# UbiquitousLearning/Mandheling-DSP-Training

Measured on AMD Instinct MI355X. Metric: training images/sec + int8 MFMA TOPS, VGG-11 batch 256, 1/2/4/8 MI355X, higher is better.
Workload: dtype int8; 1 GPU; VGG11 NITI int8 training step (fwd+relu+pool, loss grad, weight grad, input grad, SGD), 3x32x32; global_batch=256, per_gpu_batch=256, parallelism=single GPU, streams=one stream (weight gradient, then input gradient, per layer)

## Files before the change

include/niti_hip.h:

```cpp
#ifndef NITI_HIP_H
#define NITI_HIP_H

#include <stddef.h>
#include <stdint.h>

#ifdef __cplusplus
extern "C" {
#endif

enum niti_error_code {
    NITI_NO_ERROR = 0,
    NITI_OUT_OF_MEMORY = 1,
    NITI_NOT_SUPPORT = 2,
    NITI_COMPUTE_SIZE_ERROR = 3,
    NITI_NO_EXECUTION = 4,
    NITI_INVALID_VALUE = 5,
    NITI_INPUT_DATA_ERROR = 10,
    NITI_CALL_BACK_STOP = 11
};

enum niti_op_type {
    NITI_OP_CONV_INT8 = 700,
    NITI_OP_DECONV_INT8 = 701,
    NITI_OP_RELU_INT8 = 703,
// ... 157 lines not shown
    int8_t* out_p16;
    int8_t* pool3_out;
    int8_t* pool3_arg;
    int relu, pool_relu, pool_h, pool_w;
    int zero_cls, zc_h, zc_w;
    int pool3_h, pool3_w, pool3_oh, pool3_ow;
} niti_requant_fused;
int niti_requant_act_fused(const int32_t* acc, int64_t rows, int ldc, const uint32_t* amax,
                           const niti_requant_fused* f, void* stream);
int niti_requant_grad(const int32_t* acc, int64_t n, const uint32_t* amax, int rule, int8_t* g_out,
                      int8_t* w_update, void* stream);
int niti_sgd_update(const int32_t* acc, const uint32_t* amax, int rule, int co, int ci, int kk, int cip, int cop,
                    int8_t* w_ohwi16, int8_t* wt_ihwo16, int8_t* g_out, void* stream);
int niti_sgd_update_wf(const int32_t* acc, const uint32_t* amax, int rule, int co, int ci, int kk, int cip, int cop,
                       int8_t* w_ohwi16, int8_t* wt_ihwo16, int8_t* g_out, int8_t* wf, int8_t* wft, void* stream);
int niti_nhwc16_to_chwn16(const int8_t* in, int n, int hw, int cp, int np, int8_t* out, void* stream);
int niti_ohwi16_to_ihwo16(const int8_t* w, int co, int ci, int kk, int cip, int cop, int8_t* wt, void* stream);
int niti_nchw_to_nhwc16(const int8_t* x, int n, int c, int hw, int cp, int8_t* out, void* stream);
int niti_nchw_to_chwn16(const int8_t* x, int n, int c, int hw, int cp, int np, int8_t* out, void* stream);
int niti_nhwc16_to_nchw(const int8_t* x, int n, int c, int hw, int cp, int8_t* out, void* stream);
int niti_oihw_to_ohwi16(const int8_t* w, int co, int ci, int kk, int cip, int8_t* out, void* stream);
int niti_ohwi16_to_oihw(const int8_t* w, int co, int ci, int kk, int cip, int8_t* out, void* stream);
int niti_residual_add(const int8_t* a, const int8_t* ea, const int8_t* b, const int8_t* eb, int64_t n, int32_t* z,
                      int8_t* ez, uint32_t* amax, void* stream);
int niti_residual_requant(const int8_t* a, const int8_t* ea, const int8_t* b, const int8_t* eb, int64_t n,
                          const uint32_t* amax, int8_t* ez, int8_t* exp_out, int relu, int8_t* out, void* stream);
int niti_residual_requant_relu_grad(const int8_t* a, const int8_t* ea, const int8_t* b, const int8_t* eb, int64_t n,
                                    const uint32_t* amax, int8_t* ez, int8_t* exp_out, const int8_t* relu_mask,
                                    int8_t* out, void* stream);
int niti_sum_pool(const int8_t* x, int n, int hw, int cp, int32_t* acc, uint32_t* amax, void* stream);
// ... 121 lines not shown
```

mandheling-dsp-training_amd/csrc/niti_capi.hip:

```cpp
#include "../../include/niti_hip.h"
#include <memory>
#include <vector>

#include "niti_internal.hpp"
#include "niti_kernels.hpp"

struct niti_execution {
    niti::Execution* impl = nullptr;
    int op = 0;
    std::vector<void*> stage;
    std::vector<size_t> stage_bytes;
    uint32_t* err_host = nullptr;
    ~niti_execution() {
        delete impl;
        for (void* p : stage)
            if (p) (void)hipFree(p);
        if (err_host) (void)hipHostFree(err_host);
    }
};

namespace {
int code(hipError_t e) {
    if (e == hipSuccess) return NITI_NO_ERROR;
    if (e == hipErrorOutOfMemory) return NITI_OUT_OF_MEMORY;
// ... 577 lines not shown
int niti_sgd_update(const int32_t* acc, const uint32_t* amax, int rule, int co, int ci, int kk, int cip, int cop,
                    int8_t* w, int8_t* wt, int8_t* g_out, void* stream) {
    if (rule != 2 && rule != 3) return NITI_INVALID_VALUE;
    return code(niti::sgd_update(acc, amax, rule, co, ci, kk, cip, cop, w, wt, g_out, S(stream)));
}
int niti_sgd_update_wf(const int32_t* acc, const uint32_t* amax, int rule, int co, int ci, int kk, int cip, int cop,
                       int8_t* w, int8_t* wt, int8_t* g_out, int8_t* wf, int8_t* wft, void* stream) {
    if (rule != 2 && rule != 3) return NITI_INVALID_VALUE;
    if ((wf || wft) && (kk != 9 || ci % 32 != 0 || co % 32 != 0)) return NITI_NOT_SUPPORT;
    niti::SgdJob j{acc, amax, rule, co, ci, kk, cip, cop, w, wt, g_out};
    j.wf = wf;
    j.wft = wft;
    return code(niti::sgd_update_many(&j, 1, S(stream)));
}

int niti_nhwc16_to_chwn16(const int8_t* in, int n, int hw, int cp, int np, int8_t* out, void* stream) {
    return code(niti::nhwc16_to_chwn16(in, n, hw, cp, np, out, S(stream)));
}
int niti_ohwi16_to_ihwo16(const int8_t* w, int co, int ci, int kk, int cip, int cop, int8_t* wt, void* stream) {
    return code(niti::ohwi16_to_ihwo16(w, co, ci, kk, cip, cop, wt, S(stream)));
}
int niti_nchw_to_nhwc16(const int8_t* x, int n, int c, int hw, int cp, int8_t* out, void* stream) {
    return code(niti::nchw_to_nhwc16(x, n, c, hw, cp, out, S(stream)));
}
int niti_nchw_to_chwn16(const int8_t* x, int n, int c, int hw, int cp, int np, int8_t* out, void* stream) {
    return code(niti::nchw_to_chwn16(x, n, c, hw, cp, np, out, S(stream)));
}
int niti_nhwc16_to_nchw(const int8_t* x, int n, int c, int hw, int cp, int8_t* out, void* stream) {
    return code(niti::nhwc16_to_nchw(x, n, c, hw, cp, out, S(stream)));
}
// ... 215 lines not shown
```

mandheling-dsp-training_amd/csrc/niti_kernels.hip:

```cpp
#include <stdlib.h>

#include <map>
#include <atomic>
#include <mutex>
#include <type_traits>
#include <vector>
#include <algorithm>
#include <stdio.h>

#include <hip/hip_ext.h>

#include "niti_device.hpp"
#include "niti_gridbar.hpp"
#include "niti_kernels.hpp"
#include "niti_sgd.hpp"
#include "niti_map.hpp"

namespace niti {


bool ConvGeom::finalize() {
    if (n <= 0 || c_in <= 0 || h <= 0 || w <= 0 || c_out <= 0 || kh <= 0 || kw <= 0) return false;
    if (sh <= 0 || sw <= 0 || dh <= 0 || dw <= 0) return false;
    const int keh = dh * (kh - 1) + 1, kew = dw * (kw - 1) + 1;
// ... 1666 lines not shown

template <class LA, class LB, bool KT = false>
static hipError_t gemm_acc_plan(const GemmPlan& p, const LA& la, const LB& lb, int M, int N, int kc_total, int32_t* C,
                                uint32_t* amax, int32_t* ws, hipStream_t st, hipEvent_t after_gemm = nullptr,
                                SgdJob* defer = nullptr) {
    Epi e;
    if (KT) e.span = take_span();
    if (p.strat == STRAT_SLAB) {
        e.C = ws;
        e.ldc = N;
        e.slab_stride = (int64_t)slab_stride_elems(M, N);
        if (const char* f = getenv("NITI_DIAG_SPLIT_MAJOR")) e.split_major = atoi(f);
        hipError_t r = launch_mode<LA, LB, EPI_SLAB, KT>(p, la, lb, M, N, kc_total, e, st);
        if (r == hipSuccess && after_gemm != nullptr) r = hipEventRecord(after_gemm, st);
        if (r != hipSuccess) return r;
        if (defer != nullptr && ((int64_t)M * N) % 4 == 0 && (int64_t)M * N >= (int64_t)p.splits * 4096) {
            defer->slab = ws;
            defer->splits = p.splits;
            defer->slab_stride = e.slab_stride;
            defer->slab_n = (int64_t)M * N;
            return hipSuccess;
        }
        return splitk_reduce(p, ws, (int64_t)M * N, e.slab_stride, C, amax, st);
    }
    e.C = C;
    e.ldc = N;
    e.amax = amax;
    hipError_t r = launch_mode<LA, LB, EPI_STORE, KT>(p, la, lb, M, N, kc_total, e, st);
    if (r == hipSuccess && after_gemm != nullptr) r = hipEventRecord(after_gemm, st);
    return r;
}
// ... 1943 lines not shown
    const int chunks = jobs.cstart[jobs.n];
    uint32_t m = 0;
    int cur = -1;
    for (int c = blockIdx.x; c < chunks; c += gridDim.x) {
        int j = 0;
        while (j + 1 < jobs.n && c >= jobs.cstart[j + 1]) ++j;
        if (j != cur) {
            if (cur >= 0) {
                const uint32_t w = wave_max(m);
                if ((threadIdx.x & 63) == 0) publish_max(const_cast<uint32_t*>(jobs.job[cur].amax), w);
            }
            cur = j;
            m = 0;
        }
        const SgdJob& J = jobs.job[j];
        const int64_t e = (int64_t)(c - jobs.cstart[j]) * 1024 + threadIdx.x * 4;
        int64_t de = e;
        bool live = J.slab != nullptr && e < J.slab_n;
        if (live && J.slab_map == 1) {
            const uint32_t u = (uint32_t)(e >> 2);
            const uint32_t tile = u / 4608u, rem = u - tile * 4608u;
            const uint32_t row = rem / 72u, rc = rem - row * 72u;
            const uint32_t t = rc / 8u, part = rc - t * 8u;
            FastDiv ft;
            ft.m = J.tb_m;
            ft.s = J.tb_s;
            const uint32_t tco = fdiv(ft, tile), tci = tile - tco * (uint32_t)J.tb_tiles_ci;
            const int co = (int)(tco * 64u + row);
            live = co < J.co;
            de = ((int64_t)co * J.tb_ld4 + t * J.tb_cip4 + tci * 8u + part) * 4;
        }
        if (live) {
            const v4i* base = (const v4i*)(J.slab + e);
            const int64_t st4 = J.slab_stride / 4;
            v4i s = {0, 0, 0, 0};
            for (int z0 = 0; z0 < J.splits; z0 += 8) {
                v4i v[8];
#pragma unroll
                for (int q = 0; q < 8; ++q)
                    v[q] = z0 + q < J.splits ? __builtin_nontemporal_load(base + (int64_t)(z0 + q) * st4) : v4i{0, 0, 0, 0};
#pragma unroll
                for (int q = 0; q < 8; ++q) s += v[q];
            }
            *(v4i*)(const_cast<int32_t*>(J.acc) + de) = s;
#pragma unroll
            for (int q = 0; q < 4; ++q) {
                const uint32_t u = uabs32(s[q]);
                m = m > u ? m : u;
            }
        }
    }
    if (cur >= 0) {
        const uint32_t w = wave_max(m);
        if ((threadIdx.x & 63) == 0) publish_max(const_cast<uint32_t*>(jobs.job[cur].amax), w);
    }
}

__global__ void sgd_update_kernel(SgdJobs jobs, int total) {
// ... 51 lines not shown
        cin = nin;
    }
}

hipError_t sgd_combine_many(const SgdJob* jobs, int n, hipStream_t st) {
    if (n <= 0) return hipSuccess;
    if (n > SGD_MAX_JOBS) return hipErrorInvalidValue;
    SgdJobs J{};
    J.n = n;
    int chunks = 0;
    for (int i = 0; i < n; ++i) {
        J.job[i] = jobs[i];
        J.cstart[i] = chunks;
        if (jobs[i].slab != nullptr) {
            if (jobs[i].splits < 1 || jobs[i].slab_stride % 4 != 0 || jobs[i].slab_n % 4 != 0) return hipErrorInvalidValue;
            chunks += (int)((jobs[i].slab_n + 1023) / 1024);
        }
    }
    J.cstart[n] = chunks;
    if (chunks > 0) hipLaunchKernelGGL(sgd_combine_kernel, dim3(chunks < 2048 ? chunks : 2048), dim3(256), 0, st, J);
    return hipGetLastError();
}

hipError_t sgd_update_many(const SgdJob* jobs, int n, hipStream_t st) {
    if (n <= 0) return hipSuccess;
    if (n > SGD_MAX_JOBS) return hipErrorInvalidValue;
    SgdJobs J{};
    J.n = n;
    int total = 0, chunks = 0;
    for (int i = 0; i < n; ++i) {
        J.job[i] = jobs[i];
        J.start[i] = total;
        J.cstart[i] = chunks;
        total += ((jobs[i].cip + 63) / 64) * ((jobs[i].cop + 63) / 64) * jobs[i].kk;
        if (jobs[i].slab != nullptr) {
            if (jobs[i].splits < 1 || jobs[i].slab_stride % 4 != 0 || jobs[i].slab_n % 4 != 0) return hipErrorInvalidValue;
            chunks += (int)((jobs[i].slab_n + 1023) / 1024);
        }
    }
    J.cstart[n] = chunks;
    if (chunks > 0) {
        const int cgrid = chunks < 2048 ? chunks : 2048;
        hipLaunchKernelGGL(sgd_combine_kernel, dim3(cgrid), dim3(256), 0, st, J);
    }
    const int grid = total < 1536 ? total : 1536;
    hipLaunchKernelGGL(sgd_update_kernel, dim3(grid), dim3(256), 0, st, J, total);
    return hipGetLastError();
}

hipError_t sgd_update(const int32_t* acc, const uint32_t* amax, int rule, int co, int ci, int kk, int cip, int cop,
                      int8_t* w, int8_t* wT, int8_t* g_out, hipStream_t st) {
    SgdJob j{acc, amax, rule, co, ci, kk, cip, cop, w, wT, g_out};
// ... 695 lines not shown
```

mandheling-dsp-training_amd/csrc/niti_kernels.hpp:

```cpp
#pragma once

#include <hip/hip_runtime.h>
#include <stdint.h>
#include <stdlib.h>

#include "../../include/niti_hip.h"

namespace niti {

inline int round_up(int x, int m) { return (x + m - 1) / m * m; }

constexpr int MAX_SLOTS = 64;
constexpr int MAX_SLOT_STRIDE = 32;
constexpr int MAX_WORDS = MAX_SLOTS * MAX_SLOT_STRIDE;
constexpr size_t MAX_BYTES = MAX_WORDS * sizeof(uint32_t);

struct ConvGeom {
    int n, c_in, h, w;
    int c_out, kh, kw;
    int sh, sw, pt, pl, pb, pr, dh, dw;
    int oh, ow;
    int cip, cop, np;
    bool finalize();
};
// ... 317 lines not shown
    int sub_kw = 0, sub_kh = 0, sub_pt = 0, sub_pl = 0;
    const int32_t* slab = nullptr;
    int splits = 0;
    int64_t slab_stride = 0, slab_n = 0;
    int slab_map = 0;
    int tb_tiles_ci = 0, tb_cip4 = 0, tb_ld4 = 0;
    uint32_t tb_m = 0, tb_s = 0;
};
constexpr int SGD_MAX_JOBS = 24;
struct SgdJobs {
    SgdJob job[SGD_MAX_JOBS];
    int start[SGD_MAX_JOBS];
    int cstart[SGD_MAX_JOBS + 1];
    int n;
};
hipError_t sgd_update_many(const SgdJob* jobs, int n, hipStream_t st);
hipError_t sgd_combine_many(const SgdJob* jobs, int n, hipStream_t st);
bool conv_wgrad_fc_sgd_ok(const ConvGeom& g);
hipError_t conv_wgrad_fc_sgd(const ConvGeom& g, const int8_t* x, const int8_t* dy, uint32_t* amax, const SgdJob& j,
                             int pass, hipStream_t st);
hipError_t grad_exponent(const uint32_t* amax, int rule, int8_t* out, hipStream_t st);
hipError_t sgd_update(const int32_t* acc, const uint32_t* amax, int rule, int co, int ci, int kk, int cip, int cop,
                      int8_t* w, int8_t* wT, int8_t* g_out, hipStream_t st);

hipError_t maxpool_nhwc16(const int8_t* x, int n, int h, int w, int cp, int k, int s, int p, int8_t* y,
                          int oh, int ow, hipStream_t st, int8_t* arg = nullptr);
hipError_t maxpool_relu_grad_nhwc16(const int8_t* x, const int8_t* y, const int8_t* dy, int n, int h,
                                    int w, int cp, int k, int s, int p, int oh, int ow, int relu,
                                    int8_t* dx, hipStream_t st);
hipError_t relu_grad_nhwc16(const int8_t* x, const int8_t* dy, int64_t n, int8_t* out, hipStream_t st);
// ... 56 lines not shown
```

mandheling-dsp-training_amd/csrc/niti_model.hip:

```cpp
#include <stdlib.h>
#include <string.h>

#include <algorithm>
#include <array>
#include <memory>
#include <vector>

#include "../../include/niti_hip.h"
#include "niti_map.hpp"
#include "niti_step_driver.hpp"

namespace niti {

namespace {
extern int g_p16_jobs_cap;
extern int g_wgrad_batch;
}
void model_p16_jobs_cap(int cap) { g_p16_jobs_cap = cap <= 0 ? P16_MAX_JOBS : cap; }
void model_wgrad_batch(int mode) { g_wgrad_batch = mode < 0 ? 1 : mode; }

namespace {

template <int C, int KH, int KW>
struct Im2Col32 {
// ... 137 lines not shown
    std::vector<char> dp16_valid;
    std::vector<char> xp16_valid;
    void invalidate_xp16() { std::fill(xp16_valid.begin(), xp16_valid.end(), 0); }
    bool fuse_dp16 = true;
    std::vector<char> xc32_valid;
    bool fc_sgd_layer(int i) const {
        static const bool off = getenv("NITI_FC_SGD") && atoi(getenv("NITI_FC_SGD")) == 0;
        const ConvGeom& g = L[i].g;
        return in_step && !off && !dp() && !tuning && conv_wgrad_fc_sgd_ok(g) &&
               !(head_layer(i) && g.c_out <= 32 && g.cip % 32 == 0) && wgrad_p16_splits(i) == 0;
    }
    bool defer_combine() const {
        static const bool off = getenv("NITI_DIAG_SGD_COMBINE") && atoi(getenv("NITI_DIAG_SGD_COMBINE")) == 0;
        return in_step && !off && !dp() && !capturing && !tuning;
    }
    int32_t* rc_acc = nullptr;
    size_t rc_acc_size = 0;
    int8_t* gspec_alt = nullptr;
    size_t gspec_alt_bytes = 0;
    bool conv0_ranged = false;
    static bool input_fused_ok(int c_in, int k, int pad) { return input_im2col_ok(c_in, k, k) && 2 * pad < k; }
    static bool input_fused(const Layer& f) {
        const ConvGeom& o = f.og;
        return f.col && o.kh == o.kw && o.pt == o.pl && input_fused_ok(o.c_in, o.kh, o.pt) && o.sh == 1 && o.sw == 1;
    }
    bool rowconv_layer(int i) const { return use_rowconv && L[i].rc; }
    std::vector<char> dyc32_valid;
    std::vector<char> dy16_valid;
    bool rowconv_dgrad_layer(int i) const { return use_rowconv && L[i].rcd; }
    bool pool_code_layer(int i) const {
// ... 802 lines not shown
        unsigned long long* sp;
        probe_launch(i, 2, &eb, &ee, &sp);
        const bool defer = defer_combine() && s > 1 && l.slab16 != nullptr &&
                           conv_wgrad_p16_workspace(g, s) <= l.slab16_bytes;
        l.defer = SgdJob{};
        DTRY(conv_wgrad_p16(g, xp16[i], dp16[i], l.dwacc, dp ? nullptr : rng(i, 2), defer ? l.slab16 : slab_w,
                            defer ? l.slab16_bytes : slab_w_bytes, s, st, eb, ee, sp, defer ? &l.defer : nullptr));
        return NITI_NO_ERROR;
    }
    if (capturing)
        probe(i, 2, true, st);
    else
        arm_kernel_events(i, 2);
    arm_span(i, 2);
    const bool defer = defer_combine() && ensure_wslab(i);
    l.defer = SgdJob{};
    DTRY(conv_wgrad_acc(g, l.in, l.dy, l.dwacc, dp ? nullptr : rng(i, 2), defer ? l.wslab : slab_w,
                        defer ? l.wslab_bytes : slab_w_bytes, st, capturing ? probe_end_event(i, 2) : nullptr,
                        defer ? &l.defer : nullptr));
    return NITI_NO_ERROR;
}

int Model::dgrad_layer(int i, hipStream_t st) {
    const int n = batch;
    const bool dp = this->dp();
    Layer& l = L[i];
    const ConvGeom& g = l.g;
    Layer& pv = L[i - 1];
    probe(i, 1, true, st);
    if (head_dgrad_ok(i)) {
        RowConvOut o;
        o.dgrad_slot = 1;
        int8_t* next = rowconv_dgrad_layer(i - 1) && !rowconv_nhwc_pref(pv.dg) ? pv.dyc32 : nullptr;
        if (pv.pool) {
// ... 835 lines not shown
```

mandheling-dsp-training_amd/csrc/niti_resnet_model.hip:

```cpp
#include <string.h>

#include <algorithm>
#include <set>

#include "../../include/niti_hip.h"
#include "niti_map.hpp"
#include "niti_resnet_model.hpp"

namespace niti {

static ConvGeom make_geom(int n, int ci, int h, int co, int k, int s, int p) {
    ConvGeom g{};
    g.n = n;
    g.c_in = ci;
    g.h = g.w = h;
    g.c_out = co;
    g.kh = g.kw = k;
    g.sh = g.sw = s;
    g.pt = g.pl = g.pb = g.pr = p;
    g.dh = g.dw = 1;
    g.finalize();
    return g;
}

// ... 344 lines not shown
        DTRY(conv_dgrad_spec(g, c.dy, c.wT, rng(i, 1), o, slot, 1, st, alt));
    } else {
        const int8_t* subw = subpix_on() ? c.subw : nullptr;
        DTRY(conv_dgrad_phase1(g, c.dy, c.wT, acc, rng(i, 1), slab, slab_bytes, st, subw));
        if (dp && exact) DTRY(coll->allreduce(rng(i, 1), MAX_WORDS, COLL_MAX_U32, st));
        DTRY(conv_dgrad_phase2(g, c.dy, c.wT, acc, rng(i, 1), o, slab_bytes, st, subw));
    }
    probe(i, 1, false, st);
    return NITI_NO_ERROR;
}

int ResNetModel::wgrad_conv(int i, hipStream_t st) {
    RConv& c = C[i];
    probe(i, 2, true, st);
    const bool defer = in_step && !dp() && !capturing && !tuning && ensure_wslab(i);
    c.defer = SgdJob{};
    DTRY(conv_wgrad_acc(c.g, c.in, c.dy, c.dwacc, dp() ? nullptr : rng(i, 2), defer ? c.wslab : slab_w,
                        defer ? c.wslab_bytes : slab_w_bytes, st, nullptr, defer ? &c.defer : nullptr));
    probe(i, 2, false, st);
    return NITI_NO_ERROR;
}

bool ResNetModel::ensure_wslab(int i) {
    const RConv& c = C[i];
    const PlanChoice p = conv_plan_query(PLAN_WGRAD, c.g, false, slab_w_bytes);
    if (p.strat != 2 || p.splits < 2 || p.bm == PLAN_P16_TILE) return false;
    return c.wslab_bytes >= conv_wgrad_slab_bytes(c.g, p);
}

int ResNetModel::size_wslabs() {
    if (wslab_epoch == plan_override_epoch()) return NITI_NO_ERROR;
    bool synced = false;
    for (RConv& c : C) {
// ... 538 lines not shown
```

mandheling-dsp-training_amd/csrc/niti_rowconv.hip:

```cpp
#include <hip/hip_runtime.h>

#include <stdlib.h>

#include <algorithm>
#include <map>
#include <mutex>

#include "niti_device.hpp"
#include "niti_gridbar.hpp"
#include "niti_kernels.hpp"
#include "niti_map.hpp"

#ifndef RC_EXP
#define RC_EXP 0
#endif
namespace niti {

__device__ __forceinline__ int bitwidth_rc(uint32_t m) { return m <= 1u ? 0 : 32 - __clz((int)(m - 1u)); }

__device__ __forceinline__ int32_t psto_rc(int32_t a, int s) {
    const uint32_t ua = a < 0 ? 0u - (uint32_t)a : (uint32_t)a;
    const uint32_t q = ua >> s;
    const uint32_t prob = ua & ((1u << s) - 1u);
    const int h = s >> 1;
// ... 465 lines not shown
    const int8_t* px = a.pool_x + z;
    if (!pool && a.relu_mask == nullptr) return;
#pragma unroll
    for (int r = 0; r < R; ++r)
        e.y[r] = *(const v4i*)(ps + ((img * H + U.b * R + r) * W + ox) * a.cop + cb16);
    if (pool && !code) {
#pragma unroll
        for (int r = 0; r < R; ++r)
#pragma unroll
            for (int t = 0; t < 4; ++t)
                e.x[r][t] = *(const v4i*)(px + ((img * 2 * H + 2 * (U.b * R + r) + (t >> 1)) * 2 * W + 2 * ox + (t & 1)) *
                                                   a.cop + cb16);
    }
}

template <int ROWS, int WD, int G>
__device__ __forceinline__ void p16_store(const RowConvArgs& a, int lane, const int8_t* tile, int img0, int y0, int hd,
                                          int cob) {
    constexpr int PPI = ROWS * WD;
    constexpr int NROWS = G * PPI;
    static_assert(NROWS % 32 == 0 && NROWS * 32 <= RC_P16_WAVE_BYTES, "whole rounds in the wave's slot");
    const int gi = lane >> 4, j = lane & 15, chalf = gi & 1;
#pragma unroll
    for (int q = 0; q < NROWS / 32; ++q) {
        const int r0 = 16 * (2 * q + (gi >> 1));
        const int8_t* t = tile + (r0 + (j >> 1)) * 32 + 16 * chalf + 8 * (j & 1);
        const v2i lo = __builtin_amdgcn_ds_read_tr8_b64_v2i32((__attribute__((address_space(3))) v2i*)(t));
        const v2i hi = __builtin_amdgcn_ds_read_tr8_b64_v2i32((__attribute__((address_space(3))) v2i*)(t + 8 * 32));
        const int g = r0 / PPI, rem = r0 % PPI;
        const int64_t P = ((int64_t)(img0 + g) * hd + y0 + rem / WD) * WD + rem % WD;
        if (P < a.p16_pixels)
            *(v4i*)(a.p16 + ((P >> 4) * a.cop + cob * 32 + 16 * chalf + j) * 16) = v4i{lo[0], lo[1], hi[0], hi[1]};
    }
}

template <int W, int R, bool DG>
__device__ __forceinline__ void rowconv_epilogue(const RowConvArgs& a, const RowUnit<W, R>& U, int lane,
                                                 const v16i (&acc)[R], uint32_t gmax, const EpiIn<DG ? R : 1>& e,
                                                 int8_t* tile) {
    constexpr int H = W;
    const int h = lane >> 5, c = lane & 31, ox = c % W;
    const int shift = __builtin_amdgcn_readfirstlane(bitwidth_rc(gmax) - 7);
    int8_t q[R][16];
    if (shift <= 0) {
#pragma unroll
        for (int r = 0; r < R; ++r)
#pragma unroll
            for (int i = 0; i < 16; ++i) {
// ... 47 lines not shown
        }
        if constexpr (DG && R <= 4)
            if (a.p16 != nullptr) p16_store<2 * R, 2 * W, 32 / W>(a, lane, tile, U.img - c / W, 2 * U.b * R, H2, U.cob);
        return;
    }
#pragma unroll
    for (int r = 0; r < R; ++r) {
        v4i v = pack_cols(q[r]);
        const int oy = U.b * R + r;
        if (U.img_ok) {
            const int64_t po = ((img * H + oy) * W + ox) * a.cop + cb16;
            if (DG && a.relu_mask != nullptr) v &= e.y[DG ? r : 0];
            if (a.out != nullptr && (W > 1 || cb16 < a.cop)) *(v4i*)(a.out + po) = v;
            if (a.next != nullptr && a.pool_out == nullptr)
                *(v4i*)(a.next + (((img * a.COB + U.cob) * H + oy) * W + ox) * 32 + 16 * h) = v;
            if (DG && a.p16 != nullptr) *(v4i*)(tile + (((c / W) * R + r) * W + ox) * 32 + 16 * h) = v;
        }
    }
    if constexpr (DG && (R * W >= 16 || W == 2))
        if (a.p16 != nullptr) p16_store<R, W, 32 / W>(a, lane, tile, U.img - c / W, U.b * R, H, U.cob);
    if (a.pool_out != nullptr) {
        constexpr int HO = H / 2, WO = W / 2;
#pragma unroll
        for (int r = 0; r + 1 < R; r += 2) {
            int8_t pm[16];
#pragma unroll
            for (int i = 0; i < 16; ++i) {
                const int v0 = q[r][i] > q[r + 1][i] ? q[r][i] : q[r + 1][i];
                const int v1 = __builtin_amdgcn_mov_dpp(v0, 0xB1, 0xF, 0xF, false);
                pm[i] = (int8_t)(v0 > v1 ? v0 : v1);
            }
            const v4i v = pack_cols(pm);
            v4i code{0, 0, 0, 0};
            if (a.pool_code_out != nullptr) {
// ... 509 lines not shown
        if (spec && U.valid && owner) unit_epilogue<W, R, DG>(a, U, lane, acc, g_guess, ein, tile);
        if (wid == 0) {
            const int gbw = grid_bw_wait(a.bar, a.epoch, a.err, a.spin_limit, a.expect_extra, lane);
            if (a.stamps != nullptr && lane == 0) a.stamps[blockIdx.x * 64 + 9] = __builtin_amdgcn_s_memrealtime();
            const uint32_t g = gbw == 0 ? 0u : 1u << gbw;
            if (lane == 0) {
                gm = g;
                if (blockIdx.x == 0) {
                    write_exponent(a, g);
                    if (a.spec != 0) __hip_atomic_store(hint_p, (uint32_t)gbw + 1u, __ATOMIC_RELAXED, __HIP_MEMORY_SCOPE_AGENT);
                }
            }
        }
        __syncthreads();
        RC_STAMP(4);
        if (U.valid && owner && (!spec || gm != g_guess)) unit_epilogue<W, R, DG>(a, U, lane, acc, gm, ein, tile);
        RC_STAMP(5);
    } else if constexpr (MODE == RC_RANGE && W == 0) {
        uint32_t m = 0;
        seg_run<R, RC_RANGE, false>(a, lane, wid, smem, m, 0u);
        m = wave_max(m);
        if (lane == 0) red[wid] = m;
        __syncthreads();
        if (threadIdx.x == 0) publish_max(a.amax, max(max(red[0], red[1]), max(red[2], red[3])));
    } else if constexpr (MODE == RC_REQUANT && W == 0) {
        uint32_t g = 0;
        bool store = false;
        SpecBook bk{};
        if (a.spec2 == 1) {
            const int guess = spec_guess(a, false, store);
            g = guess <= 0 ? 0u : 1u << guess;
// ... 55 lines not shown
            }
            if (a.spec2 == 1 && owner) m = unit_max<W, R>(U, acc, m);
            if (store) {
                if (owner) acc_put<R>(a, wg, wid, lane, acc);
                continue;
            }
            EpiIn<DG ? R : 1> ein = {};
            if constexpr (DG) {
                if (owner) {
                    unit_prefetch<W, R>(a, U, lane, ein);
                    epi_masks<R>(a, ein);
                }
            }
            if (U.valid && owner) unit_epilogue<W, R, DG>(a, U, lane, acc, g, ein, smem + wid * RC_P16_WAVE_BYTES);
            if (DG && a.p16 != nullptr) __syncthreads();
        }
        if (a.spec2 == 1) {
            m = wave_max(m);
            if (lane == 0) red[wid] = m;
            __syncthreads();
            if (threadIdx.x == 0) publish_max(a.amax, max(max(red[0], red[1]), max(red[2], red[3])));
        }
    }
}

struct Nhwc16ToC32 {
    const int8_t* in;
    int hw, cp, cb;
    int8_t* out;
    __device__ void operator()(int64_t i) const {
// ... 164 lines not shown
    }
    if (getenv("NITI_RC_ACC_MIN_CIN") != nullptr && g.c_in < acc_min_cin()) return 0;
    int u = 0;
    const int R = rowconv_rows(g, dg, &u);
    const int G = 32 / g.w, ngb = ((g.n + G - 1) / G) * (g.h / R), ngb4 = (ngb + 3) / 4 * 4, COB = g.cop / 32;
    const int64_t wgs = rowconv_ks(g, dg) > 0 ? (int64_t)COB * ngb : (int64_t)COB * ngb4 / 4;
    return (size_t)wgs * 4 * R * 1024 * sizeof(int32_t);
}

bool rowconv_p16_ok(const ConvGeom& d, bool pool) {
    if (!rowconv_ok(d) || rowconv_seg(d)) return false;
    int u = 0;
    const int R = rowconv_rows(d, true, &u), W = d.w;
    const int64_t px = (int64_t)d.n * d.h * d.w * (pool ? 4 : 1);
    if (px % 16 != 0) return false;
    return pool || R * W >= 16 || (W == 2 && R == 2);
}

static int rowconv_ks(const ConvGeom& g, bool dg) {
    int u = 0;
    const int R = rowconv_rows(g, dg, &u);
    const int CB = (g.c_in + 31) / 32;
    if (g.w != 2 || R != 2 || CB % 4 != 0 || CB / 4 > RC_KS_MAX_NS || u >= 768) return 0;
    return CB / 4;
}

int rowconv_units(const ConvGeom& g, bool dg) {
    if (rowconv_seg(g)) return seg_plan(g).wgs * 4;
    int u = 0;
    (void)rowconv_rows(g, dg, &u);
    if (rowconv_ks(g, dg) > 0) {
// ... 381 lines not shown
```

mandheling-dsp-training_amd/niti_amd/_lib.py:

```python
from __future__ import annotations

import ctypes as C
import os
import re

_HERE = os.path.dirname(os.path.abspath(__file__))
LIB_PATH = os.environ.get("NITI_HIP_LIB") or os.path.join(_HERE, "_lib", "libniti_hip.so")
HEADER = os.path.join(os.path.dirname(os.path.dirname(_HERE)), "include", "niti_hip.h")

ERROR_NAMES = {0: "NO_ERROR", 1: "OUT_OF_MEMORY", 2: "NOT_SUPPORT", 3: "COMPUTE_SIZE_ERROR",
               4: "NO_EXECUTION", 5: "INVALID_VALUE", 10: "INPUT_DATA_ERROR", 11: "CALL_BACK_STOP"}
NOT_SUPPORT, INVALID_VALUE = 2, 5

OP_CONV_INT8 = 700
OP_DECONV_INT8 = 701
OP_RELU_INT8 = 703
OP_RELUGRAD_INT8 = 704
OP_MAXPOOL_INT8 = 705
OP_POOLGRAD_INT8 = 706
OP_LOSS_INT8 = 710
OP_LOSS_GRAD_INT8 = 711
OP_MATMUL_INT8 = 713
OP_PAD_INT8 = 714
OP_LEFTPOOLGRAD_INT8 = 718
# ... 36 lines not shown
    _fields_ = [("kernel_x", C.c_int), ("kernel_y", C.c_int), ("stride_x", C.c_int), ("stride_y", C.c_int),
                ("dilate_x", C.c_int), ("dilate_y", C.c_int), ("pad_x", C.c_int), ("pad_y", C.c_int),
                ("has_pads", C.c_int), ("pads", C.c_int * 4), ("pad_mode", C.c_int),
                ("input_count", C.c_int), ("output_count", C.c_int), ("group", C.c_int)]


class Geom(C.Structure):
    _fields_ = [(n, C.c_int) for n in (
        "n", "c_in", "h", "w", "c_out", "kh", "kw", "stride_h", "stride_w", "pad_t", "pad_l", "pad_b",
        "pad_r", "dilate_h", "dilate_w", "oh", "ow", "cip", "cop", "np")]


class WgradP16Job(C.Structure):
    _fields_ = [("g", Geom), ("x_p16", C.c_void_p), ("dy_p16", C.c_void_p), ("acc", C.c_void_p),
                ("amax", C.c_void_p)]


class ChainLayer(C.Structure):
    _fields_ = [(n, C.c_int) for n in ("c_out", "kernel", "stride", "pad", "relu", "pool", "flatten")]


class EvalTotals(C.Structure):
    _fields_ = [("images", C.c_uint64), ("top1", C.c_uint64), ("topk", C.c_uint64), ("loss_sum", C.c_double)]


class RequantFused(C.Structure):
    _fields_ = ([(n, C.c_void_p) for n in (
        "exp_in", "wscale", "exp_out", "relu_mask", "out_nhwc16", "pool_out", "pool_x", "pool_y", "pool_dx",
        "pool_dx_c32", "out_p16", "pool3_out", "pool3_arg")] + [(n, C.c_int) for n in (
            "relu", "pool_relu", "pool_h", "pool_w", "zero_cls", "zc_h", "zc_w", "pool3_h", "pool3_w", "pool3_oh",
# ... 57 lines not shown
        "niti_conv_dgrad_phase1": (ci, [C.POINTER(Geom), vp, vp, vp, vp, vp, C.c_size_t, vp]),
        "niti_conv_dgrad_phase2": (ci, [C.POINTER(Geom), vp, vp, vp, vp, vp, vp, vp, ci, vp, vp, C.c_size_t, vp]),
        "niti_nhwc16_to_p16": (ci, [vp, i64, ci, vp, vp]),
        "niti_diag_wgrad_stamps": (None, [vp]),
        "niti_diag_rowconv_stamps": (None, [vp]),
        "niti_conv_wgrad_p16_workspace": (ci, [C.POINTER(Geom), ci, C.POINTER(C.c_size_t)]),
        "niti_conv_wgrad_p16_acc": (ci, [C.POINTER(Geom), vp, vp, vp, vp, vp, C.c_size_t, ci, vp]),
        "niti_conv_wgrad_p16_many_workspace": (ci, [C.POINTER(WgradP16Job), ci, ci, ci, C.POINTER(C.c_size_t)]),
        "niti_conv_wgrad_p16_many": (ci, [C.POINTER(WgradP16Job), ci, ci, ci, vp, C.c_size_t, C.POINTER(ci), vp]),
        "niti_matmul_acc": (ci, [ci, ci, ci, vp, i64, vp, i64, vp, i64, vp, vp, C.c_size_t, vp]),
        "niti_absmax_i32": (ci, [vp, i64, vp, vp]),
        "niti_requant_act": (ci, [vp, i64, ci, vp, vp, vp, vp, ci, vp, vp, vp]),
        "niti_requant_act_fused": (ci, [vp, i64, ci, vp, C.POINTER(RequantFused), vp]),
        "niti_requant_grad": (ci, [vp, i64, vp, ci, vp, vp, vp]),
        "niti_sgd_update": (ci, [vp, vp, ci, ci, ci, ci, ci, ci, vp, vp, vp, vp]),
        "niti_nhwc16_to_chwn16": (ci, [vp, ci, ci, ci, ci, vp, vp]),
        "niti_ohwi16_to_ihwo16": (ci, [vp, ci, ci, ci, ci, ci, vp, vp]),
        "niti_nchw_to_nhwc16": (ci, [vp, ci, ci, ci, ci, vp, vp]),
        "niti_nchw_to_chwn16": (ci, [vp, ci, ci, ci, ci, ci, vp, vp]),
        "niti_nhwc16_to_nchw": (ci, [vp, ci, ci, ci, ci, vp, vp]),
        "niti_oihw_to_ohwi16": (ci, [vp, ci, ci, ci, ci, vp, vp]),
        "niti_ohwi16_to_oihw": (ci, [vp, ci, ci, ci, ci, vp, vp]),
        "niti_residual_add": (ci, [vp, vp, vp, vp, i64, vp, vp, vp, vp]),
        "niti_residual_requant": (ci, [vp, vp, vp, vp, i64, vp, vp, vp, ci, vp, vp]),
        "niti_residual_requant_relu_grad": (ci, [vp, vp, vp, vp, i64, vp, vp, vp, vp, vp, vp]),
        "niti_sum_pool": (ci, [vp, ci, ci, ci, vp, vp, vp]),
        "niti_sum_pool_grad": (ci, [vp, ci, ci, ci, vp, vp]),
        "niti_im2col": (ci, [C.POINTER(Geom), vp, ci, vp, vp]),
        "niti_im2col_nchw": (ci, [C.POINTER(Geom), vp, ci, vp, vp]),
        "niti_sgd_update_wf": (ci, [vp, vp, ci, ci, ci, ci, ci, ci, vp, vp, vp, vp, vp, vp]),
# ... 84 lines not shown
```

mandheling-dsp-training_amd/niti_amd/ops.py:

```python
from __future__ import annotations

import ctypes as C

import torch

from . import _lib as L
from ._lib import check


def _stream(stream=None):
    if stream is not None:
        return stream
    return C.c_void_p(torch.cuda.current_stream().cuda_stream)


def _ptr(t):
    return None if t is None else C.c_void_p(t.data_ptr())


def tensor(t: torch.Tensor, dims, fmt=L.FORMAT_NCHW) -> L.Tensor:
    d = list(dims) + [1] * (4 - len(dims))
    v = L.Tensor(t.data_ptr(), (C.c_int * 4)(*d), fmt)
    v._keep = t
    return v
# ... 409 lines not shown
    cop = r16(co)
    if wT is None:
        wT = torch.zeros((ci, kh, kw, cop), dtype=torch.int8, device=acc.device)
    if g is None:
        g = torch.empty(acc.shape, dtype=torch.int8, device=acc.device)
    assert wT.shape == (ci, kh, kw, cop) and g.shape == acc.shape
    if wf is not None or wft is not None:
        check(L.lib().niti_sgd_update_wf(_ptr(acc), _ptr(amax), rule, co, ci, kh * kw, cip, cop, _ptr(w16), _ptr(wT),
                                         _ptr(g), _ptr(wf), _ptr(wft), _stream(stream)), "sgd_update_wf")
        return wT, g
    check(L.lib().niti_sgd_update(_ptr(acc), _ptr(amax), rule, co, ci, kh * kw, cip, cop, _ptr(w16), _ptr(wT), _ptr(g),
                                  _stream(stream)), "sgd_update")
    return wT, g


def residual_add(a, ea, b, eb, amax, stream=None, ez=None):
    assert a.shape == b.shape and a.dtype == b.dtype == torch.int8
    z = torch.empty(a.shape, dtype=torch.int32, device=a.device)
    if ez is None:
        ez = torch.zeros(1, dtype=torch.int8, device=a.device)
    check(L.lib().niti_residual_add(_ptr(a), _ptr(ea), _ptr(b), _ptr(eb), a.numel(), _ptr(z), _ptr(ez), _ptr(amax),
                                    _stream(stream)), "residual_add")
    return z, ez


def residual_range(a, ea, b, eb, amax, stream=None):
    assert a.shape == b.shape and a.dtype == b.dtype == torch.int8
    check(L.lib().niti_residual_add(_ptr(a), _ptr(ea), _ptr(b), _ptr(eb), a.numel(), None, None, _ptr(amax),
                                    _stream(stream)), "residual_range")

# ... 160 lines not shown
```

Before: 746,300 images/s.

## Split-K slab combine across lane groups and pair-wave p16 stores for 4-wide rows

The split-K slab combine kernel now spreads the split dimension over up to 16 lanes and reduces them with xor shuffles, so small layers with many splits get more parallelism. The combine can now be deferred for any size instead of only large slabs. A tuning-time path issues the combine directly. For the W=4,R=2 row-conv case, the p16 transposed output is written through a paired-wave tile with an extra barrier, which enables the fused p16 path for that geometry. A C API and Python wrapper for the standalone combine are added. The extra barriers and shuffles add overhead, and the new lane split changes the chunk counts.

```diff
diff --git a/include/niti_hip.h b/include/niti_hip.h
--- a/include/niti_hip.h
+++ b/include/niti_hip.h
@@ -195,6 +195,15 @@
                     int8_t* w_ohwi16, int8_t* wt_ihwo16, int8_t* g_out, void* stream);
 int niti_sgd_update_wf(const int32_t* acc, const uint32_t* amax, int rule, int co, int ci, int kk, int cip, int cop,
                        int8_t* w_ohwi16, int8_t* wt_ihwo16, int8_t* g_out, int8_t* wf, int8_t* wft, void* stream);
+typedef struct niti_sgd_combine_job {
+    const int32_t* slab;
+    int splits;
+    int64_t stride;
+    int64_t n;
+    int32_t* acc;
+    uint32_t* amax;
+} niti_sgd_combine_job;
+int niti_sgd_combine(const niti_sgd_combine_job* jobs, int n_jobs, void* stream);
 int niti_nhwc16_to_chwn16(const int8_t* in, int n, int hw, int cp, int np, int8_t* out, void* stream);
 int niti_ohwi16_to_ihwo16(const int8_t* w, int co, int ci, int kk, int cip, int cop, int8_t* wt, void* stream);
 int niti_nchw_to_nhwc16(const int8_t* x, int n, int c, int hw, int cp, int8_t* out, void* stream);
diff --git a/mandheling-dsp-training_amd/csrc/niti_capi.hip b/mandheling-dsp-training_amd/csrc/niti_capi.hip
--- a/mandheling-dsp-training_amd/csrc/niti_capi.hip
+++ b/mandheling-dsp-training_amd/csrc/niti_capi.hip
@@ -615,6 +615,25 @@
     return code(niti::sgd_update_many(&j, 1, S(stream)));
 }
 
+int niti_sgd_combine(const niti_sgd_combine_job* jobs, int n_jobs, void* stream) {
+    if (!jobs || n_jobs < 1 || n_jobs > niti::SGD_MAX_JOBS) return NITI_INVALID_VALUE;
+    niti::SgdJob r[niti::SGD_MAX_JOBS];
+    for (int j = 0; j < n_jobs; ++j) {
+        const niti_sgd_combine_job& s = jobs[j];
+        if (!s.slab || !s.acc || !s.amax || s.splits < 1 || s.n < 4 || s.n % 4 || s.stride % 4 || s.stride < s.n)
+            return NITI_INVALID_VALUE;
+        if (((uintptr_t)s.slab | (uintptr_t)s.acc) & 15) return NITI_INVALID_VALUE;
+        r[j] = niti::SgdJob{};
+        r[j].acc = s.acc;
+        r[j].amax = s.amax;
+        r[j].slab = s.slab;
+        r[j].splits = s.splits;
+        r[j].slab_stride = s.stride;
+        r[j].slab_n = s.n;
+    }
+    return code(niti::sgd_combine_many(r, n_jobs, S(stream)));
+}
+
 int niti_nhwc16_to_chwn16(const int8_t* in, int n, int hw, int cp, int np, int8_t* out, void* stream) {
     return code(niti::nhwc16_to_chwn16(in, n, hw, cp, np, out, S(stream)));
 }
diff --git a/mandheling-dsp-training_amd/csrc/niti_kernels.hip b/mandheling-dsp-training_amd/csrc/niti_kernels.hip
--- a/mandheling-dsp-training_amd/csrc/niti_kernels.hip
+++ b/mandheling-dsp-training_amd/csrc/niti_kernels.hip
@@ -1704,7 +1704,7 @@
         hipError_t r = launch_mode<LA, LB, EPI_SLAB, KT>(p, la, lb, M, N, kc_total, e, st);
         if (r == hipSuccess && after_gemm != nullptr) r = hipEventRecord(after_gemm, st);
         if (r != hipSuccess) return r;
-        if (defer != nullptr && ((int64_t)M * N) % 4 == 0 && (int64_t)M * N >= (int64_t)p.splits * 4096) {
+        if (defer != nullptr && ((int64_t)M * N) % 4 == 0) {
             defer->slab = ws;
             defer->splits = p.splits;
             defer->slab_stride = e.slab_stride;
@@ -3678,7 +3678,9 @@
             m = 0;
         }
         const SgdJob& J = jobs.job[j];
-        const int64_t e = (int64_t)(c - jobs.cstart[j]) * 1024 + threadIdx.x * 4;
+        const int G = sgd_combine_lanes(J.splits, J.slab_n);
+        const int g = threadIdx.x & (G - 1);
+        const int64_t e = ((int64_t)(c - jobs.cstart[j]) * (256 / G) + threadIdx.x / G) * 4;
         int64_t de = e;
         bool live = J.slab != nullptr && e < J.slab_n;
         if (live && J.slab_map == 1) {
@@ -3694,18 +3696,26 @@
             live = co < J.co;
             de = ((int64_t)co * J.tb_ld4 + t * J.tb_cip4 + tci * 8u + part) * 4;
         }
+        v4i s = {0, 0, 0, 0};
         if (live) {
             const v4i* base = (const v4i*)(J.slab + e);
             const int64_t st4 = J.slab_stride / 4;
-            v4i s = {0, 0, 0, 0};
-            for (int z0 = 0; z0 < J.splits; z0 += 8) {
+            for (int z0 = g; z0 < J.splits; z0 += 8 * G) {
                 v4i v[8];
 #pragma unroll
-                for (int q = 0; q < 8; ++q)
-                    v[q] = z0 + q < J.splits ? __builtin_nontemporal_load(base + (int64_t)(z0 + q) * st4) : v4i{0, 0, 0, 0};
+                for (int q = 0; q < 8; ++q) {
+                    const int z = z0 + q * G;
+                    v[q] = z < J.splits ? __builtin_nontemporal_load(base + (int64_t)z * st4) : v4i{0, 0, 0, 0};
+                }
 #pragma unroll
                 for (int q = 0; q < 8; ++q) s += v[q];
             }
+        }
+        for (int o = G >> 1; o > 0; o >>= 1) {
+#pragma unroll
+            for (int q = 0; q < 4; ++q) s[q] += __shfl_xor(s[q], o, 64);
+        }
+        if (live && g == 0) {
             *(v4i*)(const_cast<int32_t*>(J.acc) + de) = s;
 #pragma unroll
             for (int q = 0; q < 4; ++q) {
@@ -3787,7 +3797,7 @@
         J.cstart[i] = chunks;
         if (jobs[i].slab != nullptr) {
             if (jobs[i].splits < 1 || jobs[i].slab_stride % 4 != 0 || jobs[i].slab_n % 4 != 0) return hipErrorInvalidValue;
-            chunks += (int)((jobs[i].slab_n + 1023) / 1024);
+            chunks += sgd_combine_chunks(jobs[i].splits, jobs[i].slab_n);
         }
     }
     J.cstart[n] = chunks;
@@ -3808,7 +3818,7 @@
         total += ((jobs[i].cip + 63) / 64) * ((jobs[i].cop + 63) / 64) * jobs[i].kk;
         if (jobs[i].slab != nullptr) {
             if (jobs[i].splits < 1 || jobs[i].slab_stride % 4 != 0 || jobs[i].slab_n % 4 != 0) return hipErrorInvalidValue;
-            chunks += (int)((jobs[i].slab_n + 1023) / 1024);
+            chunks += sgd_combine_chunks(jobs[i].splits, jobs[i].slab_n);
         }
     }
     J.cstart[n] = chunks;
diff --git a/mandheling-dsp-training_amd/csrc/niti_kernels.hpp b/mandheling-dsp-training_amd/csrc/niti_kernels.hpp
--- a/mandheling-dsp-training_amd/csrc/niti_kernels.hpp
+++ b/mandheling-dsp-training_amd/csrc/niti_kernels.hpp
@@ -355,6 +355,17 @@
     int cstart[SGD_MAX_JOBS + 1];
     int n;
 };
+static_assert(sizeof(SgdJobs) <= 4096, "SgdJobs is passed by value: the kernel-argument limit");
+__host__ __device__ inline int sgd_combine_lanes(int splits, int64_t slab_n) {
+    if (slab_n >= (int64_t)splits * 4096) return 1;
+    int G = 1;
+    while (G < 16 && G * 2 <= splits && (slab_n / 4) * G < 131072) G <<= 1;
+    return G;
+}
+inline int sgd_combine_chunks(int splits, int64_t slab_n) {
+    const int per = 256 / sgd_combine_lanes(splits, slab_n);
+    return (int)((slab_n / 4 + per - 1) / per);
+}
 hipError_t sgd_update_many(const SgdJob* jobs, int n, hipStream_t st);
 hipError_t sgd_combine_many(const SgdJob* jobs, int n, hipStream_t st);
 bool conv_wgrad_fc_sgd_ok(const ConvGeom& g);
diff --git a/mandheling-dsp-training_amd/csrc/niti_model.hip b/mandheling-dsp-training_amd/csrc/niti_model.hip
--- a/mandheling-dsp-training_amd/csrc/niti_model.hip
+++ b/mandheling-dsp-training_amd/csrc/niti_model.hip
@@ -175,6 +175,10 @@
         static const bool off = getenv("NITI_DIAG_SGD_COMBINE") && atoi(getenv("NITI_DIAG_SGD_COMBINE")) == 0;
         return in_step && !off && !dp() && !capturing && !tuning;
     }
+    bool in_step_combine() const {
+        static const bool off = getenv("NITI_DIAG_SGD_COMBINE") && atoi(getenv("NITI_DIAG_SGD_COMBINE")) == 0;
+        return !off && !dp();
+    }
     int32_t* rc_acc = nullptr;
     size_t rc_acc_size = 0;
     int8_t* gspec_alt = nullptr;
@@ -1007,10 +1011,19 @@
         arm_kernel_events(i, 2);
     arm_span(i, 2);
     const bool defer = defer_combine() && ensure_wslab(i);
+    const bool tune_defer = tuning && in_step_combine() &&
+                            conv_plan_query(PLAN_WGRAD, g, false, slab_w_bytes).bm != PLAN_TAPS_TILE;
     l.defer = SgdJob{};
     DTRY(conv_wgrad_acc(g, l.in, l.dy, l.dwacc, dp ? nullptr : rng(i, 2), defer ? l.wslab : slab_w,
                         defer ? l.wslab_bytes : slab_w_bytes, st, capturing ? probe_end_event(i, 2) : nullptr,
-                        defer ? &l.defer : nullptr));
+                        defer || tune_defer ? &l.defer : nullptr));
+    if (tune_defer && l.defer.slab != nullptr) {
+        SgdJob j = l.defer;
+        j.acc = l.dwacc;
+        j.amax = rng(i, 2);
+        l.defer = SgdJob{};
+        if (sgd_combine_many(&j, 1, st) != hipSuccess) return NITI_NO_EXECUTION;
+    }
     return NITI_NO_ERROR;
 }
 
diff --git a/mandheling-dsp-training_amd/csrc/niti_resnet_model.hip b/mandheling-dsp-training_amd/csrc/niti_resnet_model.hip
--- a/mandheling-dsp-training_amd/csrc/niti_resnet_model.hip
+++ b/mandheling-dsp-training_amd/csrc/niti_resnet_model.hip
@@ -382,9 +382,18 @@
     RConv& c = C[i];
     probe(i, 2, true, st);
     const bool defer = in_step && !dp() && !capturing && !tuning && ensure_wslab(i);
+    const bool tune_defer = tuning && !dp() &&
+                            conv_plan_query(PLAN_WGRAD, c.g, false, slab_w_bytes).bm != PLAN_TAPS_TILE;
     c.defer = SgdJob{};
     DTRY(conv_wgrad_acc(c.g, c.in, c.dy, c.dwacc, dp() ? nullptr : rng(i, 2), defer ? c.wslab : slab_w,
-                        defer ? c.wslab_bytes : slab_w_bytes, st, nullptr, defer ? &c.defer : nullptr));
+                        defer ? c.wslab_bytes : slab_w_bytes, st, nullptr, defer || tune_defer ? &c.defer : nullptr));
+    if (tune_defer && c.defer.slab != nullptr) {
+        SgdJob j = c.defer;
+        j.acc = c.dwacc;
+        j.amax = rng(i, 2);
+        c.defer = SgdJob{};
+        if (sgd_combine_many(&j, 1, st) != hipSuccess) return NITI_NO_EXECUTION;
+    }
     probe(i, 2, false, st);
     return NITI_NO_ERROR;
 }
diff --git a/mandheling-dsp-training_amd/csrc/niti_rowconv.hip b/mandheling-dsp-training_amd/csrc/niti_rowconv.hip
--- a/mandheling-dsp-training_amd/csrc/niti_rowconv.hip
+++ b/mandheling-dsp-training_amd/csrc/niti_rowconv.hip
@@ -503,15 +503,17 @@
     }
 }
 
-template <int ROWS, int WD, int G>
+template <int ROWS, int WD, int G, int NQ = G * ROWS * WD / 32>
 __device__ __forceinline__ void p16_store(const RowConvArgs& a, int lane, const int8_t* tile, int img0, int y0, int hd,
-                                          int cob) {
+                                          int cob, int q0 = 0) {
     constexpr int PPI = ROWS * WD;
     constexpr int NROWS = G * PPI;
     static_assert(NROWS % 32 == 0 && NROWS * 32 <= RC_P16_WAVE_BYTES, "whole rounds in the wave's slot");
+    static_assert(NQ >= 1 && NQ <= NROWS / 32, "rounds of the tile");
     const int gi = lane >> 4, j = lane & 15, chalf = gi & 1;
 #pragma unroll
-    for (int q = 0; q < NROWS / 32; ++q) {
+    for (int qq = 0; qq < NQ; ++qq) {
+        const int q = q0 + qq;
         const int r0 = 16 * (2 * q + (gi >> 1));
         const int8_t* t = tile + (r0 + (j >> 1)) * 32 + 16 * chalf + 8 * (j & 1);
         const v2i lo = __builtin_amdgcn_ds_read_tr8_b64_v2i32((__attribute__((address_space(3))) v2i*)(t));
@@ -521,6 +523,17 @@
         if (P < a.p16_pixels)
             *(v4i*)(a.p16 + ((P >> 4) * a.cop + cob * 32 + 16 * chalf + j) * 16) = v4i{lo[0], lo[1], hi[0], hi[1]};
     }
+}
+
+template <int W, int R, bool DG>
+constexpr bool RC_P16_PAIR = DG && W == 4 && R == 2;
+template <int W, int R>
+__device__ __forceinline__ int8_t* p16_pair_tile(const RowUnit<W, R>& U, int8_t* own) {
+    return own - U.b * RC_P16_WAVE_BYTES;
+}
+template <int W, int R>
+__device__ __forceinline__ void p16_pair_store(const RowConvArgs& a, const RowUnit<W, R>& U, int lane, int8_t* own) {
+    p16_store<4, 4, 8, 2>(a, lane, p16_pair_tile<W, R>(U, own), U.img - (lane & 31) / W, 0, 4, U.cob, 2 * U.b);
 }
 
 template <int W, int R, bool DG>
@@ -598,10 +611,15 @@
             if (a.out != nullptr && (W > 1 || cb16 < a.cop)) *(v4i*)(a.out + po) = v;
             if (a.next != nullptr && a.pool_out == nullptr)
                 *(v4i*)(a.next + (((img * a.COB + U.cob) * H + oy) * W + ox) * 32 + 16 * h) = v;
-            if (DG && a.p16 != nullptr) *(v4i*)(tile + (((c / W) * R + r) * W + ox) * 32 + 16 * h) = v;
-        }
-    }
-    if constexpr (DG && (R * W >= 16 || W == 2))
+            if constexpr (RC_P16_PAIR<W, R, DG>) {
+                if (a.p16 != nullptr)
+                    *(v4i*)(p16_pair_tile<W, R>(U, tile) + (((c / W) * H + oy) * W + ox) * 32 + 16 * h) = v;
+            } else {
+                if (DG && a.p16 != nullptr) *(v4i*)(tile + (((c / W) * R + r) * W + ox) * 32 + 16 * h) = v;
+            }
+        }
+    }
+    if constexpr (DG && !RC_P16_PAIR<W, R, DG> && (R * W >= 16 || W == 2))
         if (a.p16 != nullptr) p16_store<R, W, 32 / W>(a, lane, tile, U.img - c / W, U.b * R, H, U.cob);
     if (a.pool_out != nullptr) {
         constexpr int HO = H / 2, WO = W / 2;
@@ -1141,7 +1159,14 @@
         }
         __syncthreads();
         RC_STAMP(4);
-        if (U.valid && owner && (!spec || gm != g_guess)) unit_epilogue<W, R, DG>(a, U, lane, acc, gm, ein, tile);
+        const bool redo = !spec || gm != g_guess;
+        if (U.valid && owner && redo) unit_epilogue<W, R, DG>(a, U, lane, acc, gm, ein, tile);
+        if constexpr (RC_P16_PAIR<W, R, DG>) {
+            if (a.p16 != nullptr && a.pool_dx == nullptr) {
+                if (redo) __syncthreads();
+                if (U.valid) p16_pair_store<W, R>(a, U, lane, tile);
+            }
+        }
         RC_STAMP(5);
     } else if constexpr (MODE == RC_RANGE && W == 0) {
         uint32_t m = 0;
@@ -1227,6 +1252,12 @@
             }
             if (U.valid && owner) unit_epilogue<W, R, DG>(a, U, lane, acc, g, ein, smem + wid * RC_P16_WAVE_BYTES);
             if (DG && a.p16 != nullptr) __syncthreads();
+            if constexpr (RC_P16_PAIR<W, R, DG>) {
+                if (a.p16 != nullptr && a.pool_dx == nullptr) {
+                    if (U.valid) p16_pair_store<W, R>(a, U, lane, smem + wid * RC_P16_WAVE_BYTES);
+                    __syncthreads();
+                }
+            }
         }
         if (a.spec2 == 1) {
             m = wave_max(m);
@@ -1421,7 +1452,7 @@
     const int R = rowconv_rows(d, true, &u), W = d.w;
     const int64_t px = (int64_t)d.n * d.h * d.w * (pool ? 4 : 1);
     if (px % 16 != 0) return false;
-    return pool || R * W >= 16 || (W == 2 && R == 2);
+    return pool || R * W >= 16 || (W == 2 && R == 2) || (W == 4 && R == 2);
 }
 
 static int rowconv_ks(const ConvGeom& g, bool dg) {
diff --git a/mandheling-dsp-training_amd/niti_amd/_lib.py b/mandheling-dsp-training_amd/niti_amd/_lib.py
--- a/mandheling-dsp-training_amd/niti_amd/_lib.py
+++ b/mandheling-dsp-training_amd/niti_amd/_lib.py
@@ -74,6 +74,11 @@
 class WgradP16Job(C.Structure):
     _fields_ = [("g", Geom), ("x_p16", C.c_void_p), ("dy_p16", C.c_void_p), ("acc", C.c_void_p),
                 ("amax", C.c_void_p)]
+
+
+class SgdCombineJob(C.Structure):
+    _fields_ = [("slab", C.c_void_p), ("splits", C.c_int), ("stride", C.c_int64), ("n", C.c_int64),
+                ("acc", C.c_void_p), ("amax", C.c_void_p)]
 
 
 class ChainLayer(C.Structure):
@@ -161,6 +166,7 @@
         "niti_requant_act_fused": (ci, [vp, i64, ci, vp, C.POINTER(RequantFused), vp]),
         "niti_requant_grad": (ci, [vp, i64, vp, ci, vp, vp, vp]),
         "niti_sgd_update": (ci, [vp, vp, ci, ci, ci, ci, ci, ci, vp, vp, vp, vp]),
+        "niti_sgd_combine": (ci, [C.POINTER(SgdCombineJob), ci, vp]),
         "niti_nhwc16_to_chwn16": (ci, [vp, ci, ci, ci, ci, vp, vp]),
         "niti_ohwi16_to_ihwo16": (ci, [vp, ci, ci, ci, ci, ci, vp, vp]),
         "niti_nchw_to_nhwc16": (ci, [vp, ci, ci, ci, ci, vp, vp]),
diff --git a/mandheling-dsp-training_amd/niti_amd/ops.py b/mandheling-dsp-training_amd/niti_amd/ops.py
--- a/mandheling-dsp-training_amd/niti_amd/ops.py
+++ b/mandheling-dsp-training_amd/niti_amd/ops.py
@@ -447,6 +447,15 @@
     return wT, g
 
 
+def sgd_combine(jobs, stream=None):
+    arr = (L.SgdCombineJob * len(jobs))()
+    for j, (slab, n, acc, amax) in enumerate(jobs):
+        assert slab.dtype == torch.int32 and slab.dim() == 2 and slab.is_contiguous() and acc.numel() >= n
+        arr[j].slab, arr[j].splits, arr[j].stride, arr[j].n = slab.data_ptr(), slab.shape[0], slab.shape[1], n
+        arr[j].acc, arr[j].amax = acc.data_ptr(), amax.data_ptr()
+    check(L.lib().niti_sgd_combine(arr, len(jobs), _stream(stream)), "sgd_combine")
+
+
 def residual_add(a, ea, b, eb, amax, stream=None, ez=None):
     assert a.shape == b.shape and a.dtype == b.dtype == torch.int8
     z = torch.empty(a.shape, dtype=torch.int32, device=a.device)
```

After: 755,300 images/s (median of 6 runs). 1.2% higher.
